# rayglover-ibm/sparse-solvers

Measured on AMD Instinct MI355X. Metric: signals recovered/sec (Homotopy l1, m=8192 n=65536 k=64 fp32), higher is better.
Workload: dtype f32; 1 GPU; configs[1]: one signal per solve, A 8192x65536 fp32 = default_rng(1234).standard_normal/sqrt(m) (SURVEY 8d recipe), k=64 positive coefficients, tol 1e-3, max_iter 256; shipped defaults (reference behaviour: tie_guard 0, zero_on_removal 0); m=8192, n=65536, k=64, sweep_variant=5, engine=1

## Files before the change

### sparse-solvers_amd/csrc/resident.hip

```cpp
#include "ss_hip_internal.h"
#include "ss_hip_device.h"
#include "resident.h"

#include <hip/hip_fp16.h>

#include <algorithm>
#include <cmath>
#include <cstdio>
#include <cstdlib>
#include <cstring>

namespace sship {

template <typename T> struct ResVec;
template <> struct ResVec<double> { typedef double v2 __attribute__((ext_vector_type(2))); };
template <> struct ResVec<float>  { typedef float v2 __attribute__((ext_vector_type(2))); };

template <typename T>
struct ResLds {
    T* I;
    T* dvec;
    T* xvec;
    T* u1sg;
    T* u2w;
    int32_t* posof;
    uint32_t* subc;
    uint32_t* pcol;
    uint32_t* psub;
};

template <typename T>
__host__ __device__ inline size_t res_lds_bytes()
{
    typedef ResCfg<T> C;
    return ((size_t)C::PCAP * (C::PCAP + 1) + 6 * (size_t)C::PCAP) * sizeof(T) + ((size_t)2 * C::S + 2 * (size_t)C::PCAP) * 4;
}

template <typename T> __device__ __forceinline__ T res_sqrt(T v);
template <> __device__ __forceinline__ float res_sqrt<float>(float v) { return sqrtf(v); }
template <> __device__ __forceinline__ double res_sqrt<double>(double v) { return sqrt(v); }
template <typename T> __device__ __forceinline__ T res_fma(T a, T b, T c);
template <> __device__ __forceinline__ float res_fma<float>(float a, float b, float c) { return __builtin_fmaf(a, b, c); }
template <> __device__ __forceinline__ double res_fma<double>(double a, double b, double c) { return __builtin_fma(a, b, c); }
template <typename T> __device__ __forceinline__ T res_abs(T v) { return v < T(0) ? -v : v; }

__device__ __forceinline__ uint32_t uni(uint32_t v) { return (uint32_t)__builtin_amdgcn_readfirstlane((int)v); }
__device__ __forceinline__ int32_t uni(int32_t v) { return __builtin_amdgcn_readfirstlane(v); }
__device__ __forceinline__ float uni(float v) { return __uint_as_float(uni(__float_as_uint(v))); }
__device__ __forceinline__ double uni(double v)
{
    const uint32_t lo = uni((uint32_t)__double2loint(v)), hi = uni((uint32_t)__double2hiint(v));
    return __hiloint2double((int)hi, (int)lo);
}

__device__ __forceinline__ void lds_barrier() { asm volatile("s_waitcnt lgkmcnt(0)\n\ts_barrier" ::: "memory"); }

__device__ __forceinline__ void cmov_inplace(float& dst, float src, unsigned long long msk)
{
    asm volatile("v_cndmask_b32_e64 %0, %0, %1, %2" : "+v"(dst) : "v"(src), "s"(msk));
}
__device__ __forceinline__ void cmov_inplace(double& dst, double src, unsigned long long msk)
{
    uint32_t lo = (uint32_t)__double2loint(dst), hi = (uint32_t)__double2hiint(dst);
    const uint32_t slo = (uint32_t)__double2loint(src), shi = (uint32_t)__double2hiint(src);
    asm volatile("v_cndmask_b32_e64 %0, %0, %2, %4\n\tv_cndmask_b32_e64 %1, %1, %3, %4" : "+v"(lo), "+v"(hi) : "v"(slo), "v"(shi), "s"(msk));
    dst = __hiloint2double((int)hi, (int)lo);
}

template <typename T>
__device__ __forceinline__ T group8_sum(T v)
{
    v += dpp_mov<kDppXor1>(v);
    v += dpp_mov<kDppXor2>(v);
    v += dpp_mov<kDppHalfMirror>(v);
    return v;
}

template <typename T>
__device__ __forceinline__ T wave_max_val(T v)
{
    { const T o = dpp_mov<kDppXor1>(v); v = o > v ? o : v; }
    { const T o = dpp_mov<kDppXor2>(v); v = o > v ? o : v; }
    { const T o = dpp_mov<kDppHalfMirror>(v); v = o > v ? o : v; }
    { const T o = dpp_mov<kDppMirror>(v); v = o > v ? o : v; }
    T b = lane_value(v, 0);
#pragma unroll
    for (int r = 1; r < 4; ++r) { const T o = lane_value(v, 16 * r); b = o > b ? o : b; }
    return b;
}

template <typename T, bool OMP, bool STAMPS = false>
__global__ __launch_bounds__(ResCfg<T>::THREADS)
void k_res_solve(const T* __restrict__ Gs_all, uint32_t gpitch, size_t g_slot_stride, const T* __restrict__ c0_all, uint32_t c0_stride,
                 const uint32_t* __restrict__ sub_all, uint32_t n, T tol, uint32_t max_iter, int strict_sign, int tie_guard, int tie_exit,
                 uint32_t kcap, uint32_t* __restrict__ log_hdr, T* __restrict__ log_H, uint32_t* __restrict__ log_pcol, T* __restrict__ log_X, T* __restrict__ log_D,
                 T* __restrict__ x_all, uint32_t x_stride, uint32_t* __restrict__ gam2_all, uint32_t* __restrict__ touched2_all,
                 DevState* __restrict__ st_all, TraceEntry* trace, uint32_t trace_cap, unsigned long long* dbg = nullptr)
{
    unsigned long long tph[6] = { 0, 0, 0, 0, 0, 0 };
    unsigned long long tlast = 0;
#define RES_STAMP(PH) if constexpr (STAMPS) { const unsigned long long now_ = __builtin_readcyclecounter(); tph[PH] += now_ - tlast; tlast = now_; }
    typedef ResCfg<T> C;
    typedef typename ResVec<T>::v2 V2;
    constexpr uint32_t S = C::S, THREADS = C::THREADS, PCAP = C::PCAP, LOGCAP = C::LOGCAP;
    constexpr int CT = C::CT, PT = C::PCAP / 8;
    constexpr uint32_t NW = (THREADS + 63) / 64;
    constexpr uint32_t IP = PCAP + 1u;
    static_assert(THREADS / 8 * CT == S, "eight lanes per column group");
    static_assert(PCAP % 8 == 0 && (CT == 4 || CT == 8), "positions dealt out over the eight lanes of a group");
    extern __shared__ __attribute__((aligned(16))) unsigned char smem[];
    __shared__ T s_max[16];
    __shared__ T s_minv[16];
    __shared__ uint32_t s_mini[16];
    __shared__ T s_f[4];
    __shared__ uint32_t s_tie;
    ResLds<T> L;
    {
        T* p = reinterpret_cast<T*>(smem);
        L.I = p; p += (size_t)PCAP * IP;
        L.dvec = p; p += PCAP; L.xvec = p; p += PCAP; L.u1sg = p; p += 2 * PCAP; L.u2w = p; p += 2 * PCAP;
        L.posof = reinterpret_cast<int32_t*>(p);
        L.subc = reinterpret_cast<uint32_t*>(L.posof + S);
        L.pcol = L.subc + S;
        L.psub = L.pcol + PCAP;
    }
    const uint32_t slot = blockIdx.x, t = threadIdx.x, lane = t & 63u, wave = t >> 6;
    const uint32_t grp = t >> 3, g = t & 7u;
    const T* Gs = Gs_all + (size_t)slot * g_slot_stride;
    const T* c0 = c0_all + (size_t)slot * c0_stride;
    const uint32_t* sub = sub_all + (size_t)slot * S;
    T* x_out = x_all + (size_t)slot * x_stride;
    uint32_t* gam_out = gam2_all + (size_t)slot * 2 * kcap;
    uint32_t* tch_out = touched2_all + (size_t)slot * 2 * kcap;
    DevState* st = st_all + slot;
    uint32_t* hdr = log_hdr + (size_t)slot * LOGCAP * 8;
    T* LH = log_H != nullptr ? log_H + (size_t)slot * LOGCAP * 2 : nullptr;
    T* LX = log_X + (size_t)slot * LOGCAP * PCAP;
    T* LD = log_D != nullptr ? log_D + (size_t)slot * LOGCAP * PCAP : nullptr;
    if (slot != 0) trace = nullptr;

    const uint32_t jc0 = grp * (uint32_t)CT;
    const bool owner = g < (uint32_t)CT;
    const uint32_t myj = jc0 + (g & (uint32_t)(CT - 1));
    const uint32_t mycol = sub[myj];
    const bool myvalid = owner && mycol < n;
    const T my_c0 = mycol < n ? c0[mycol] : T(0);
    T my_c = my_c0, my_q = T(0);
    T gr[CT][PT];
#pragma unroll
    for (int c = 0; c < CT; ++c)
#pragma unroll
        for (int e = 0; e < PT; ++e) gr[c][e] = T(0);
    for (uint32_t j = t; j < S; j += THREADS) { L.subc[j] = sub[j]; L.posof[j] = -1; }
    for (uint32_t p = t; p < PCAP; p += THREADS) {
        L.dvec[p] = T(0); L.xvec[p] = T(0); L.pcol[p] = 0xffffffffu; L.psub[p] = 0u;
        L.u1sg[2 * p] = T(0); L.u1sg[2 * p + 1] = T(0); L.u2w[2 * p] = T(0); L.u2w[2 * p + 1] = T(0);
    }
    for (uint32_t e = t; e < PCAP * IP; e += THREADS) L.I[e] = T(0);
    if (t == 0) s_tie = 0u;
    T warm = T(0);
    {
        const size_t gbytes = (size_t)S * gpitch * sizeof(T);
        const unsigned char* gb = reinterpret_cast<const unsigned char*>(Gs);
#pragma unroll 4
        for (size_t off = (size_t)t * 128u; off < gbytes; off += (size_t)THREADS * 128u) warm += *reinterpret_cast<const T*>(gb + off);
    }

    auto wave_first = [&](T v, T ext, uint32_t idx) __attribute__((always_inline)) -> uint32_t {
        const unsigned long long bal = __builtin_amdgcn_ballot_w64(v == ext);
        const int src = bal != 0ull ? (int)__builtin_ctzll(bal) : 0;
        return (uint32_t)__builtin_amdgcn_readlane((int)idx, src);
    };
    auto block_min = [&](T& v, uint32_t& i) __attribute__((always_inline)) {
        const T wv = -wave_max_val<T>(-v);
        const uint32_t wi = wave_first(v, wv, i);
        if (lane == 0) { s_minv[wave] = wv; s_mini[wave] = wi; }
        lds_barrier();
        T bv = s_minv[0];
        uint32_t bi = s_mini[0];
#pragma unroll
        for (uint32_t w = 1; w < NW; ++w) {
            const T ov = s_minv[w];
            const uint32_t oi = s_mini[w];
            if (ov < bv) { bv = ov; bi = oi; }
        }
        v = uni(bv); i = uni(bi);
    };
    auto block_argmax = [&](T& v, uint32_t& i) __attribute__((always_inline)) {
        const T wv = wave_max_val<T>(v);
        const uint32_t wi = wave_first(v, wv, i);
        lds_barrier();
        if (lane == 0) { s_minv[wave] = wv; s_mini[wave] = wi; }
        lds_barrier();
        T bv = s_minv[0];
        uint32_t bi = s_mini[0];
#pragma unroll
        for (uint32_t w = 1; w < NW; ++w) {
            const T ov = s_minv[w];
            const uint32_t oi = s_mini[w];
            if (ov > bv) { bv = ov; bi = oi; }
        }
        v = uni(bv); i = uni(bi);
        lds_barrier();
    };
    auto border_inverse = [&](uint32_t P, T dvv) __attribute__((always_inline)) {
        constexpr uint32_t RW = PCAP / 2u + 1u;
        constexpr uint32_t NG = THREADS / RW;
        const uint32_t Pn = P + 1u;
        const uint32_t pa = t % RW, vg = t / RW;
        const uint32_t a0 = pa, a1 = Pn - 1u - pa;
        if (P != 0xffffffffu && vg < NG && 2u * pa < Pn + 1u - 0u && a0 <= a1) {
            const uint32_t n0 = Pn - a0;
            const uint32_t ntot = a0 == a1 ? n0 : n0 + (Pn - a1);
            const T u0 = a0 < P ? L.u2w[2 * a0] : T(0), u1v = a1 < P ? L.u2w[2 * a1] : T(0);
#pragma nounroll
            for (uint32_t k = vg; k < ntot; k += NG) {
                const bool first = k < n0;
                const uint32_t a = first ? a0 : a1;
                const uint32_t b = first ? a0 + k : a1 + (k - n0);
                const T ua = first ? u0 : u1v;
                T val;
                if (b == P) val = a == P ? dvv : -dvv * ua;
                else val = L.I[a * IP + b] + (dvv * ua) * L.u2w[2 * b];
                L.I[a * IP + b] = val;
                L.I[b * IP + a] = val;
            }
        }
    };

    auto enter_row = [&](uint32_t spi, uint32_t Pn, uint32_t pendP, T pend_dv) __attribute__((always_inline)) -> T {
        const T* row = Gs + (size_t)spi * gpitch;
        const T mine_g = row[myj];
        T gv[CT];
        if constexpr (sizeof(T) == 8) {
            const v2d a = *reinterpret_cast<const v2d*>(row + jc0), b = *reinterpret_cast<const v2d*>(row + jc0 + 2);
            gv[0] = a[0]; gv[1] = a[1]; gv[2] = b[0]; gv[3] = b[1];
        } else {
            const v4f a = *reinterpret_cast<const v4f*>(row + jc0), b = *reinterpret_cast<const v4f*>(row + jc0 + 4);
#pragma unroll
            for (int e = 0; e < 4; ++e) { gv[e] = a[e]; gv[4 + e] = b[e]; }
        }
        border_inverse(pendP, pend_dv);
        const uint32_t e_new = uni(Pn >> 3);
        const unsigned long long msk = __builtin_amdgcn_ballot_w64(g == (Pn & 7u));
#pragma unroll
        for (int e = 0; e < PT; ++e) {
            if (e_new == (uint32_t)e) {
#pragma unroll
                for (int c = 0; c < CT; ++c) cmov_inplace(gr[c][e], gv[c], msk);
            }
        }
        return mine_g;
    };
    auto chain = [&](const T* vec, uint32_t P) __attribute__((always_inline)) -> T {
        T acc[CT];
#pragma unroll
        for (int c = 0; c < CT; ++c) acc[c] = T(0);
#pragma unroll
        for (int e = 0; e < PT; ++e) {
            if ((uint32_t)(8 * e) < P) {
                const T dval = vec[8 * e + (int)g];
#pragma unroll
                for (int c = 0; c < CT; ++c) acc[c] = res_fma<T>(dval, gr[c][e], acc[c]);
            }
        }
        T h4[4];
        if constexpr (CT == 8) {
            const bool up = (g & 4u) != 0u;
#pragma unroll
            for (int i = 0; i < 4; ++i) {
                const T keep = up ? acc[4 + i] : acc[i], send = up ? acc[i] : acc[4 + i];
                h4[i] = keep + dpp_mov<kDppHalfMirror>(send);
            }
        } else {
#pragma unroll
            for (int i = 0; i < 4; ++i) h4[i] = acc[i] + dpp_mov<kDppHalfMirror>(acc[i]);
        }
        const bool b1 = (g & 2u) != 0u, b0 = (g & 1u) != 0u;
        const T k0 = (b1 ? h4[2] : h4[0]) + dpp_mov<kDppXor2>(b1 ? h4[0] : h4[2]);
        const T k1 = (b1 ? h4[3] : h4[1]) + dpp_mov<kDppXor2>(b1 ? h4[1] : h4[3]);
        return (b0 ? k1 : k0) + dpp_mov<kDppXor1>(b0 ? k0 : k1);
    };
    auto inverse_pass = [&](uint32_t P) __attribute__((always_inline)) {
        constexpr int CH = sizeof(T) == 8 ? 6 : PT;
        for (uint32_t a = grp; a < P; a += THREADS / 8u) {
            const T* row = L.I + (size_t)a * IP + g;
            const T* us = L.u1sg + 2u * g;
            T s1 = T(0), s2 = T(0);
#pragma nounroll
            for (int e0 = 0; e0 < PT; e0 += CH) {
                if ((uint32_t)(8 * e0) < P) {
                    T iv[CH];
                    V2 pr[CH];
#pragma unroll
                    for (int e = 0; e < CH; ++e) {
                        if (e0 + e < PT) {
                            iv[e] = row[8 * (e0 + e)];
                            pr[e] = *reinterpret_cast<const V2*>(&us[16 * (e0 + e)]);
                        } else { iv[e] = T(0); pr[e] = V2{ T(0), T(0) }; }
                    }
#pragma unroll
                    for (int e = 0; e < CH; ++e) {
                        s1 = res_fma<T>(iv[e], pr[e][0], s1);
                        s2 = res_fma<T>(iv[e], pr[e][1], s2);
                    }
                }
            }
            s1 = group8_sum<T>(s1); s2 = group8_sum<T>(s2);
            if (g == 0) { L.u2w[2 * a] = s1; L.u2w[2 * a + 1] = s2; }
        }
    };
    auto two_dots = [&](uint32_t P, T& d1, T& d2) __attribute__((always_inline)) {
        T a1 = T(0), a2 = T(0);
#pragma nounroll
        for (uint32_t b = lane; b < P; b += 64u) {
            const V2 pr = *reinterpret_cast<const V2*>(&L.u1sg[2 * b]);
            const T u2b = L.u2w[2 * b];
            a1 = res_fma<T>(pr[0], u2b, a1);
            a2 = res_fma<T>(u2b, pr[1], a2);
        }
        d1 = wave_sum<T>(a1); d2 = wave_sum<T>(a2);
    };
    uint32_t P = 0, status = 0, iter = 0, nlog = 0, reason = 0;
    T c_inf = T(0), lambda_prev = T(0), gamma_prev = T(0), lambda0 = T(0);
    int32_t mypos = -1;
    bool tie_any = false;
    lds_barrier();

    uint32_t sp0;
    {
        T bv = myvalid ? res_abs<T>(my_c) : T(-1);
        uint32_t bi = myvalid ? myj : 0xffffffffu;
        block_argmax(bv, bi);
        sp0 = bi;
        lambda0 = bv;
    }
    if (sp0 >= S) { status = kStatusSubsetDecline; reason |= kReasonNoCand; }
    else {
        const T g00 = enter_row(sp0, 0u, 0xffffffffu, T(0));
        if (owner && myj == sp0) {
            const T nrm = res_sqrt<T>(g00);
            const T inv00 = T(1) / (nrm * nrm);
            const T seed = strict_sign ? my_c : res_abs<T>(my_c);
            const T sg0 = sign_tol<T>(seed, tol);
            L.I[0] = inv00;
            if (OMP) L.xvec[0] = inv00 * my_c; else L.dvec[0] = inv00 * sg0;
            L.pcol[0] = mycol; L.psub[0] = sp0; L.posof[sp0] = 0;
            mypos = 0;
            if (!OMP && trace != nullptr) { trace[0].idx = mycol; trace[0].added = 1; trace[0].gamma = 0.0; trace[0].c_inf = (double)res_abs<T>(my_c); }
        }
        P = 1;
        c_inf = lambda0;
        lambda_prev = lambda0;
        if (!((double)tol >= (sizeof(T) == 8 ? kGramGuard64 : kGramGuard) * (double)lambda0)) { status = kStatusSubsetDecline; reason |= kReasonGuard; }
        lds_barrier();
    }

    if constexpr (OMP) {
        if (status == 0u && !(lambda0 > tol)) { status = kStatusSubsetDecline; reason |= kReasonNoCand; }
        if (status == 0u) {
            if (t == 0) {
                uint32_t* h = hdr;
                h[0] = 0u; h[1] = 1u; h[2] = L.subc[sp0]; h[3] = 1u; h[4] = __float_as_uint((float)lambda0); h[5] = 0u; h[6] = 0xffffffffu; h[7] = 0u;
                if (LH != nullptr) { LH[0] = lambda0; LH[1] = T(0); }
                if (trace != nullptr && 1u < trace_cap) { trace[1].idx = L.subc[sp0]; trace[1].added = 1u; trace[1].gamma = 0.0; trace[1].c_inf = (double)lambda0; }
            }
            if (t < PCAP) LX[t] = T(0);
            nlog = 1;
            iter = 1;
        }
        for (uint32_t round = 2; status == 0u; ++round) {
            my_c = my_c0 - chain(L.xvec, P);
            T bv = T(-1);
            uint32_t bi = 0xffffffffu;
            if (myvalid) { bv = res_abs<T>(my_c); bi = myj; }
            block_argmax(bv, bi);
            c_inf = bv;
            const bool stop = !(c_inf > tol) || round > max_iter;
            const bool logfull = nlog >= LOGCAP;
            const uint32_t spi = bi < S ? bi : 0u;
            const bool stall = !stop && (bi >= S || uni(L.posof[spi]) >= 0);
            const bool full = !stop && (P >= PCAP || P + 1u > kcap);
            const bool ok = !stop && !logfull && !stall && !full;
            if (logfull) { status = kStatusSubsetDecline; reason |= kReasonLog; }
            else if (stall) { status = kStatusSubsetDecline; reason |= kReasonNoCand; }
            else if (full) { status = kStatusSubsetDecline; reason |= kReasonPositions; }
            else if (stop) { status = 0xffffffffu; iter = round - 1; }
            const uint32_t idx = uni(L.subc[spi]);
            if (!logfull) {
                if (t == 0) {
                    uint32_t* h = hdr + nlog * 8;
                    h[0] = P; h[1] = stop ? 0u : 1u; h[2] = ok ? idx : 0xffffffffu; h[3] = ok ? 1u : 0u; h[4] = __float_as_uint((float)c_inf); h[5] = 0u;
                    h[6] = 0xffffffffu; h[7] = 0u;
                    if (LH != nullptr) { LH[nlog * 2] = c_inf; LH[nlog * 2 + 1] = T(0); }
                    if (ok && trace != nullptr && round < trace_cap) { trace[round].idx = idx; trace[round].added = 1u; trace[round].gamma = 0.0; trace[round].c_inf = (double)c_inf; }
                }
                if (t < PCAP) LX[(size_t)nlog * PCAP + t] = t < P ? L.xvec[t] : T(0);
                ++nlog;
            }
            const T my_g = enter_row(spi, ok ? P : 0xffffffffu, 0xffffffffu, T(0));
            if (owner && mypos >= 0) { L.u1sg[2 * mypos] = my_g; L.u1sg[2 * mypos + 1] = my_c0; }
            if (ok && owner && myj == spi) { s_f[0] = my_g; s_f[1] = my_c0; L.posof[spi] = (int32_t)P; L.pcol[P] = idx; L.psub[P] = spi; mypos = (int32_t)P; }
            lds_barrier();
            inverse_pass(P);
            lds_barrier();
            T d1, d2;
            two_dots(P, d1, d2);
            const T dvv = T(1) / (s_f[0] - d1);
            const T beta = dvv * (s_f[1] - d2);
            if (ok && t < P) L.xvec[t] = L.u2w[2 * t + 1] - beta * L.u2w[2 * t];
            if (ok && t == P) L.xvec[P] = beta;
            border_inverse(ok ? P : 0xffffffffu, dvv);
            lds_barrier();
            if (ok) { P += 1u; iter = round; }
        }
        if (status == 0xffffffffu) status = 0u;
    } else {
        if (status == 0u) my_q = chain(L.dvec, P);
        uint32_t pendP = 0xffffffffu;
        T pend_dv = T(0);
        for (uint32_t round = 1; status == 0u; ++round) {
            if constexpr (STAMPS) tlast = __builtin_readcyclecounter();
            const bool stop = (round > 1 && !(c_inf > tol)) || round > max_iter;
            const bool logfull = nlog >= LOGCAP;
            const bool in_band = tie_band<T>(c_inf, lambda_prev, gamma_prev, lambda0);
            T m = Lim<T>::max();
            bool tie = false;
            if (myvalid) {
                if (mypos >= 0) {
                    const T tt = -L.xvec[mypos] / L.dvec[mypos];
                    if (tt > T(0) && tt < m) m = tt;
                } else {
                    const T dl = T(1) - my_q, dr = T(1) + my_q;
                    if (dl != T(0)) {
                        T tt = (c_inf - my_c) / dl;
                        if (tie_guard && tt == T(0) && dl > T(0)) tt = Lim<T>::tiny();
                        if (tt == T(0) && in_band) tie = true;
                        if (tt > T(0) && tt < m) m = tt;
                    }
                    if (dr != T(0)) {
                        T tt = (c_inf + my_c) / dr;
                        if (tie_guard && tt == T(0) && dr > T(0)) tt = Lim<T>::tiny();
                        if (tt == T(0) && in_band) tie = true;
                        if (tt > T(0) && tt < m) m = tt;
                    }
                }
            }
            if (tie) s_tie = 1u;
            T gmm = m;
            uint32_t bi = myvalid ? myj : 0xffffffffu;
            block_min(gmm, bi);
            RES_STAMP(0)
            if (!stop) tie_any = uni(s_tie) != 0u || tie_any;
            const uint32_t spi = bi < S ? bi : 0u;
            const bool tied = !stop && tie_any && tie_exit != 0;
            const bool nocand = !stop && !tied && (bi >= S || !(gmm < Lim<T>::max()));
            const bool leaves = !stop && !tied && !nocand && uni(L.posof[spi]) >= 0;
            const bool full = !stop && !tied && !nocand && !leaves && (P >= PCAP || P + 1u > kcap);
            const bool ok = !stop && !logfull && !tied && !nocand && !leaves && !full;
            if (logfull) { status = kStatusSubsetDecline; reason |= kReasonLog; }
            else if (stop) { status = 0xffffffffu; iter = round - 1; }
            else if (tied) { status = kStatusTieRerun; reason |= kReasonTie; iter = round - 1; }
            else if (nocand) { status = kStatusSubsetDecline; reason |= kReasonNoCand; }
            else if (leaves) { status = kStatusSubsetDecline; reason |= kReasonRemoval; }
            else if (full) { status = kStatusSubsetDecline; reason |= kReasonPositions; }
            const uint32_t idx = uni(L.subc[spi]);
            if (!logfull) {
                if (t == 0) {
                    uint32_t* h = hdr + nlog * 8;
                    h[0] = P; h[1] = stop ? 0u : 1u; h[2] = ok ? idx : 0xffffffffu; h[3] = ok ? 1u : 0u; h[4] = __float_as_uint((float)c_inf);
                    h[5] = ok ? __float_as_uint((float)gmm) : 0u; h[6] = 0xffffffffu; h[7] = in_band ? 1u : 0u;
                    if (LH != nullptr) { LH[nlog * 2] = c_inf; LH[nlog * 2 + 1] = ok ? gmm : T(0); }
                    if (ok && trace != nullptr && round < trace_cap) { trace[round].idx = idx; trace[round].added = 1u; trace[round].gamma = (double)gmm; trace[round].c_inf = (double)c_inf; }
                }
                if (t < PCAP) {
                    LX[(size_t)nlog * PCAP + t] = t < P ? L.xvec[t] : T(0);
                    if (LD != nullptr) LD[(size_t)nlog * PCAP + t] = t < P ? L.dvec[t] : T(0);
                }
                if (stop || tied || ok) ++nlog;
            }
            const T my_g = enter_row(spi, ok ? P : 0xffffffffu, pendP, pend_dv);
            pendP = 0xffffffffu;
            if (ok && t < P) L.xvec[t] = L.xvec[t] + gmm * L.dvec[t];
            if (ok) my_c = res_fma<T>(-gmm, my_q, my_c);
            {
                const T mx = wave_max_val<T>(myvalid ? res_abs<T>(my_c) : T(-1));
                if (lane == 0) s_max[wave] = mx;
            }
            if (owner && mypos >= 0) { L.u1sg[2 * mypos] = my_g; L.u1sg[2 * mypos + 1] = sign_tol<T>(my_c, tol); }
            if (ok && owner && myj == spi) {
                s_f[0] = my_g; s_f[1] = sign_tol<T>(my_c, tol);
                L.posof[spi] = (int32_t)P; L.pcol[P] = idx; L.psub[P] = spi; mypos = (int32_t)P;
            }
            lds_barrier();
            RES_STAMP(1)
            T c_next = s_max[0];
#pragma unroll
            for (uint32_t w = 1; w < NW; ++w) { const T o = s_max[w]; c_next = o > c_next ? o : c_next; }
            c_next = uni(c_next);
            if (t == 0) s_tie = 0u;
            inverse_pass(P);
            lds_barrier();
            RES_STAMP(2)
            T d1, d2;
            two_dots(P, d1, d2);
            const T dvv = T(1) / (s_f[0] - d1);
            const T beta = dvv * (s_f[1] - d2);
            if (ok && t < P) L.dvec[t] = L.u2w[2 * t + 1] - beta * L.u2w[2 * t];
            if (ok && t == P) L.dvec[P] = beta;
            pendP = ok ? P : 0xffffffffu;
            pend_dv = dvv;
            lds_barrier();
            RES_STAMP(3)
            if (ok) {
                P += 1u;
                lambda_prev = c_inf;
                gamma_prev = gmm;
                c_inf = c_next;
                iter = round;
            }
            my_q = chain(L.dvec, P);
            RES_STAMP(4)
            if constexpr (STAMPS) tph[5] += 1;
        }
        if (status == 0xffffffffu) status = 0u;
    }
    if constexpr (STAMPS) {
        if (dbg != nullptr && slot == 0u && t == 0u)
            for (int q = 0; q < 6; ++q) dbg[q] = tph[q];
    }
#undef RES_STAMP
    lds_barrier();
    if (t < PCAP) log_pcol[(size_t)slot * PCAP + t] = t < P ? L.pcol[t] : 0xffffffffu;
    if (status == 0u || status == kStatusTieRerun) {
        if (t < P) {
            const uint32_t col = L.pcol[t];
            uint32_t rk = 0;
#pragma nounroll
            for (uint32_t b = 0; b < P; ++b) rk += L.pcol[b] < col ? 1u : 0u;
            gam_out[rk] = col;
            tch_out[rk] = col;
            x_out[col] = L.xvec[t];
        }
    }
    if (t == 0) {
        st->done = 1;
        st->status = status;
        st->iter = iter;
        st->K = P;
        st->ntouched = P;
        st->cur = 0;
        st->c_inf = (double)c_inf;
        st->gamma = (double)gamma_prev;
        st->tie_stall = tie_any ? 1u : 0u;
        st->lambda0 = (float)lambda0;
        st->solo_nlog = nlog;
        st->need_sweep = 0;
        st->done_round = iter + 1u;
        st->sub_reason = reason;
    }
    if (warm == T(1.2345e-30)) st->pad4_[0] = 1u;
}

constexpr uint32_t kG64T = 64, kG64Step = 32, kG64Pitch = kG64Step + 1;
typedef double res_v4d __attribute__((ext_vector_type(4)));

__global__ __launch_bounds__(256)
void k_sgram64_part(const double* __restrict__ At, uint32_t ldm, uint32_t n, const uint32_t* __restrict__ sub, uint32_t rows_per,
                    double* __restrict__ part)
{
    constexpr uint32_t S = ResCfg<double>::S;
    __shared__ double sI[kG64T][kG64Pitch];
    __shared__ double sJ[kG64T][kG64Pitch];
    sub += (size_t)blockIdx.z * S;
    part += (size_t)blockIdx.z * gridDim.y * S * S;
    const uint32_t b = blockIdx.x;
    uint32_t tt = (uint32_t)((__fsqrt_rn(8.f * (float)b + 1.f) - 1.f) * 0.5f);
    while (tt * (tt + 1u) / 2u > b) --tt;
    while ((tt + 1u) * (tt + 2u) / 2u <= b) ++tt;
    const uint32_t bj = tt, bi = b - tt * (tt + 1u) / 2u;
    const uint32_t chunk = blockIdx.y;
    const uint32_t tid = threadIdx.x, lane = tid & 63u, w = tid >> 6;
    const uint32_t wi = w >> 1, wj = w & 1u;
    const uint32_t sc = tid >> 2, sq = tid & 3u;
    const uint32_t ci = sub[bi * kG64T + sc], cj = sub[bj * kG64T + sc];
    const bool oki = ci < n, okj = cj < n;
    const double* gi = At + (size_t)(oki ? ci : 0u) * ldm + (size_t)chunk * rows_per + 8u * sq;
    const double* gj = At + (size_t)(okj ? cj : 0u) * ldm + (size_t)chunk * rows_per + 8u * sq;
    const v2d zero2 = { 0.0, 0.0 };
    v2d vi[4], vj[4];
#define SG64_LOAD(R0)                                                                         \
    _Pragma("unroll") for (int p = 0; p < 4; ++p) {                                           \
        vi[p] = oki ? *reinterpret_cast<const v2d*>(gi + (R0) + 2 * p) : zero2;               \
        vj[p] = okj ? *reinterpret_cast<const v2d*>(gj + (R0) + 2 * p) : zero2;               \
    }
    SG64_LOAD(0u)
    res_v4d acc[2][2];
#pragma unroll
    for (int i = 0; i < 2; ++i)
#pragma unroll
        for (int j = 0; j < 2; ++j) acc[i][j] = res_v4d{ 0.0, 0.0, 0.0, 0.0 };
    const uint32_t l15 = lane & 15u, kq = lane >> 4;
    for (uint32_t r0 = 0; r0 < rows_per; r0 += kG64Step) {
        __syncthreads();
#pragma unroll
        for (int p = 0; p < 4; ++p) {
            sI[sc][8u * sq + 2u * (uint32_t)p] = vi[p][0]; sI[sc][8u * sq + 2u * (uint32_t)p + 1u] = vi[p][1];
            sJ[sc][8u * sq + 2u * (uint32_t)p] = vj[p][0]; sJ[sc][8u * sq + 2u * (uint32_t)p + 1u] = vj[p][1];
        }
        __syncthreads();
        if (r0 + kG64Step < rows_per) SG64_LOAD(r0 + kG64Step)
#pragma unroll
        for (uint32_t k4 = 0; k4 < kG64Step; k4 += 4) {
            const double a0 = sI[32u * wi + l15][k4 + kq], a1 = sI[32u * wi + 16u + l15][k4 + kq];
            const double b0 = sJ[32u * wj + l15][k4 + kq], b1 = sJ[32u * wj + 16u + l15][k4 + kq];
            acc[0][0] = __builtin_amdgcn_mfma_f64_16x16x4f64(a0, b0, acc[0][0], 0, 0, 0);
            acc[0][1] = __builtin_amdgcn_mfma_f64_16x16x4f64(a0, b1, acc[0][1], 0, 0, 0);
            acc[1][0] = __builtin_amdgcn_mfma_f64_16x16x4f64(a1, b0, acc[1][0], 0, 0, 0);
            acc[1][1] = __builtin_amdgcn_mfma_f64_16x16x4f64(a1, b1, acc[1][1], 0, 0, 0);
        }
    }
#undef SG64_LOAD
    double* Pp = part + (size_t)chunk * S * S;
#pragma unroll
    for (int i = 0; i < 2; ++i)
#pragma unroll
        for (int j = 0; j < 2; ++j)
#pragma unroll
            for (int e = 0; e < 4; ++e) {
                const uint32_t row = bi * kG64T + 32u * wi + 16u * (uint32_t)i + 4u * (uint32_t)e + kq;
                const uint32_t col = bj * kG64T + 32u * wj + 16u * (uint32_t)j + l15;
                Pp[(size_t)row * S + col] = acc[i][j][e];
                if (bi != bj) Pp[(size_t)col * S + row] = acc[i][j][e];
            }
}

__global__ __launch_bounds__(256)
void k_sgram64_sum(const double* __restrict__ part, uint32_t nsplit, double* __restrict__ gs, const double* __restrict__ At, uint32_t ldm,
                   const double* __restrict__ y, const uint32_t* __restrict__ sub, uint32_t n, double* __restrict__ c0, uint32_t c0_stride)
{
    constexpr uint32_t S = ResCfg<double>::S;
    constexpr uint32_t NB = S * S / 256u;
    {
        const size_t slot = blockIdx.y;
        part += slot * nsplit * S * S; gs += slot * S * S; y += slot * ldm; sub += slot * S; c0 += slot * c0_stride;
    }
    if (blockIdx.x >= NB) {
        __shared__ double sv[16];
        const uint32_t col = sub[blockIdx.x - NB];
        const double* a = At + (size_t)(col < n ? col : 0u) * ldm;
        double acc = 0.0;
        for (uint32_t r0 = 2u * threadIdx.x; r0 < ldm; r0 += 8u * 512u) {
            v2d av[8], yv[8];
// ... 78 lines not shown
    }
    const uint32_t Pfin = hdr[(size_t)(nlog - 1u) * 8u];
    if (tid < kR64Rhs) {
        float sc = 1.f;
        if (tid < nst) {
            const double lam = LH[(size_t)(tid + 1u) * 2u];
            const bool final_state = !(hdr[(size_t)(tid + 1u) * 8u + 1u] & 1u);
            sc = res_state_scale((float)(final_state ? fmax(lam, tol) : lam));
        }
        sS[tid] = sc;
    }
    const uint32_t rg = tid & 15u, sgp = tid >> 4;
    double acc[3][4][4];
    {
        const v2d y0 = *reinterpret_cast<const v2d*>(y + r0 + 4u * rg), y1 = *reinterpret_cast<const v2d*>(y + r0 + 4u * rg + 2u);
#pragma unroll
        for (int rd = 0; rd < 3; ++rd)
#pragma unroll
            for (int si = 0; si < 4; ++si) { acc[rd][si][0] = y0[0]; acc[rd][si][1] = y0[1]; acc[rd][si][2] = y1[0]; acc[rd][si][3] = y1[1]; }
    }
    for (uint32_t u0 = 0; u0 < Pfin; u0 += 16u) {
        __syncthreads();
        {
            const uint32_t p = tid >> 4, q4 = tid & 15u;
            const uint32_t u = u0 + p;
            const uint32_t col = u < Pfin ? pcol[u] : 0xffffffffu;
            v2d a0 = { 0.0, 0.0 }, a1 = { 0.0, 0.0 };
            if (col < n) {
                a0 = *reinterpret_cast<const v2d*>(At + (size_t)col * ldm + r0 + 4u * q4);
                a1 = *reinterpret_cast<const v2d*>(At + (size_t)col * ldm + r0 + 4u * q4 + 2u);
            }
            *reinterpret_cast<v2d*>(&sAc[p][4u * q4]) = a0;
            *reinterpret_cast<v2d*>(&sAc[p][4u * q4 + 2u]) = a1;
            for (uint32_t e = tid; e < 16u * XP; e += 256u) {
                const uint32_t k = e / 16u, pp = e - k * 16u;
                sXt[pp][k] = (u0 + pp < Pfin && k < nst) ? LX[(size_t)(k + 1u) * PCAP + u0 + pp] : 0.0;
            }
        }
        __syncthreads();
#pragma unroll
        for (int rd = 0; rd < 3; ++rd) {
            const uint32_t s0 = 64u * (uint32_t)rd + 4u * sgp;
            if (s0 < nst) {
#pragma unroll 4
                for (uint32_t p = 0; p < 16u; ++p) {
                    const v2d a0 = *reinterpret_cast<const v2d*>(&sAc[p][4u * rg]), a1 = *reinterpret_cast<const v2d*>(&sAc[p][4u * rg + 2u]);
                    const v2d x0 = *reinterpret_cast<const v2d*>(&sXt[p][s0]), x1 = *reinterpret_cast<const v2d*>(&sXt[p][s0 + 2u]);
                    const double av[4] = { a0[0], a0[1], a1[0], a1[1] }, xv[4] = { x0[0], x0[1], x1[0], x1[1] };
#pragma unroll
                    for (int si = 0; si < 4; ++si)
#pragma unroll
                        for (int ri = 0; ri < 4; ++ri) acc[rd][si][ri] = __builtin_fma(-xv[si], av[ri], acc[rd][si][ri]);
                }
            }
        }
    }
    bool ovf = false;
#pragma unroll
    for (int rd = 0; rd < 3; ++rd) {
#pragma unroll
        for (int si = 0; si < 4; ++si) {
            const uint32_t kk = 64u * (uint32_t)rd + 4u * sgp + (uint32_t)si;
            const float sc = sS[kk < kR64Rhs ? kk : 0u];
            float ss = 0.f;
            __half hv[4];
#pragma unroll
            for (int ri = 0; ri < 4; ++ri) {
                const float r = (float)acc[rd][si][ri];
                ss = __builtin_fmaf(r, r, ss);
                const float v = r * sc;
                if (kk < nst && !(fabsf(v) < 60000.f)) ovf = true;
                hv[ri] = __float2half_rn(v);
            }
            ss += __shfl_xor(ss, 1); ss += __shfl_xor(ss, 2); ss += __shfl_xor(ss, 4); ss += __shfl_xor(ss, 8);
            if (kk < nst) {
                *reinterpret_cast<uint2*>(r16 + (size_t)kk * ldm + r0 + 4u * rg) = *reinterpret_cast<const uint2*>(hv);
                if (rg == 0u) rn2p[(size_t)blockIdx.x * kR64Rhs + kk] = ss * 1.0001f;
            }
        }
    }
    if (ovf && !scan) { __hip_atomic_store(&st->need_sweep, 1u, __ATOMIC_RELAXED, __HIP_MEMORY_SCOPE_AGENT); atomicOr(&st->sub_reason, kReasonOverflow); }
    if (blockIdx.x == 0u) {
        if (tid == 0u && blockIdx.y == 0u) *headroom = __float_as_uint(ratio0);
        if (tid < nst) {
            const uint32_t* hh = hdr + (size_t)(tid + 1u) * 8u;
            const uint32_t* hp = hdr + (size_t)tid * 8u;
            const double lam_d = LH[(size_t)(tid + 1u) * 2u];
            const double lam_pd = LH[(size_t)tid * 2u], gam_pd = LH[(size_t)tid * 2u + 1u];
            const float lam = (float)lam_d;
            const bool final_state = !(hh[1] & 1u);
            const float slack = 1e-12f * (float)LH[0];
            float bound;
            if (omp) {
                bound = (final_state && !(lam_d > tol) ? (float)tol * 0.9375f : lam * 0.875f) - slack;
            } else {
                const double lam_exp = lam_pd - gam_pd;
                const bool ls_jump = final_state && !(lam_d > tol) && !(lam_exp > 1e-13 * LH[0]);
                if (ls_jump) bound = (float)tol * 0.9375f - slack;
                else bound = fminf(lam, (float)lam_exp) * 0.875f - slack;
                const bool irregular = hp[3] == 0u || lam_d > lam_pd * (1.0 + 1e-12);
                if (irregular && !scan) {
                    bound = -1.f;
                    atomicOr(&st->sub_reason, kReasonIrregular);
                    __hip_atomic_store(&st->need_sweep, 1u, __ATOMIC_RELAXED, __HIP_MEMORY_SCOPE_AGENT);
                }
                if (scan && (irregular || final_state)) bound = 3.0e38f;
            }
            const float inv_sk = 1.f / sS[tid];
            tab[tid * 4u + 0] = meta[1] * inv_sk;
            tab[tid * 4u + 1] = bound;
            tab[tid * 4u + 2] = inv_sk;
            tab[tid * 4u + 3] = lam;
        }
    }
}

template <typename T>
bool res_solve_usable()
{
    static const bool ok = [] {
        const hipError_t e = hipFuncSetAttribute(reinterpret_cast<const void*>(&k_res_solve<T, false>), hipFuncAttributeMaxDynamicSharedMemorySize,
                                                 (int)res_lds_bytes<T>());
        const hipError_t e2 = hipFuncSetAttribute(reinterpret_cast<const void*>(&k_res_solve<T, true>), hipFuncAttributeMaxDynamicSharedMemorySize,
                                                  (int)res_lds_bytes<T>());
        if (e != hipSuccess || e2 != hipSuccess) (void)hipGetLastError();
        return e == hipSuccess && e2 == hipSuccess;
    }();
    return ok;
}
template bool res_solve_usable<float>();
template bool res_solve_usable<double>();

template <typename T>
hipError_t launch_res_solve(ss_hip_ctx* ctx, uint32_t nslots, const T* Gs, uint32_t gpitch, size_t g_slot_stride, const T* c0, uint32_t c0_stride,
                            const uint32_t* sub, T tol, uint32_t max_iter, uint32_t kcap, const ResLog<T>& log, T* x, uint32_t x_stride,
                            uint32_t* gam2, uint32_t* touched2, DevState* st, TraceEntry* trace, uint32_t trace_cap, bool omp)
{
    if (!res_solve_usable<T>()) return hipErrorInvalidConfiguration;
    static unsigned long long* dbg = nullptr;
    static const bool stamps = std::getenv("SS_HIP_RES_STAMPS") != nullptr;
    if (stamps && !omp) {
        static const bool ok = [] {
            const bool a = hipFuncSetAttribute(reinterpret_cast<const void*>(&k_res_solve<T, false, true>), hipFuncAttributeMaxDynamicSharedMemorySize,
                                               (int)res_lds_bytes<T>()) == hipSuccess;
            return a && hipMalloc(&dbg, 8 * sizeof(unsigned long long)) == hipSuccess;
        }();
        if (ok) {
            hipLaunchKernelGGL((k_res_solve<T, false, true>), dim3(nslots), dim3(ResCfg<T>::THREADS), res_lds_bytes<T>(), ctx->stream, Gs, gpitch, g_slot_stride, c0, c0_stride,
                               sub, (uint32_t)ctx->n, tol, max_iter, ctx->strict_sign, ctx->tie_guard, (ctx->tie_rerun && !ctx->tie_guard) ? 1 : 0, kcap,
                               log.hdr, log.H, log.pcol, log.X, log.D, x, x_stride, gam2, touched2, st, trace, trace_cap, dbg);
            unsigned long long tp[6];
            if (hipMemcpyAsync(tp, dbg, sizeof(tp), hipMemcpyDeviceToHost, ctx->stream) == hipSuccess && hipStreamSynchronize(ctx->stream) == hipSuccess) {
                const double r = tp[5] ? (double)tp[5] : 1.0;
                std::fprintf(stderr, "[k_res_solve<%s>, cycles per round over %llu rounds] scan+argmin %.0f  row+x+c %.0f  inverse pass %.0f  dots+dir+border %.0f  chain %.0f\n",
                             sizeof(T) == 8 ? "double" : "float", tp[5], tp[0] / r, tp[1] / r, tp[2] / r, tp[3] / r, tp[4] / r);
            }
            return hipGetLastError();
        }
    }
    if (omp)
        hipLaunchKernelGGL((k_res_solve<T, true>), dim3(nslots), dim3(ResCfg<T>::THREADS), res_lds_bytes<T>(), ctx->stream, Gs, gpitch, g_slot_stride, c0, c0_stride,
                           sub, (uint32_t)ctx->n, tol, max_iter, ctx->strict_sign, ctx->tie_guard, (ctx->tie_rerun && !ctx->tie_guard) ? 1 : 0, kcap,
                           log.hdr, log.H, log.pcol, log.X, log.D, x, x_stride, gam2, touched2, st, trace, trace_cap);
    else
        hipLaunchKernelGGL((k_res_solve<T, false>), dim3(nslots), dim3(ResCfg<T>::THREADS), res_lds_bytes<T>(), ctx->stream, Gs, gpitch, g_slot_stride, c0, c0_stride,
                           sub, (uint32_t)ctx->n, tol, max_iter, ctx->strict_sign, ctx->tie_guard, (ctx->tie_rerun && !ctx->tie_guard) ? 1 : 0, kcap,
                           log.hdr, log.H, log.pcol, log.X, log.D, x, x_stride, gam2, touched2, st, trace, trace_cap);
    return hipGetLastError();
}
template hipError_t launch_res_solve<float>(ss_hip_ctx*, uint32_t, const float*, uint32_t, size_t, const float*, uint32_t, const uint32_t*, float, uint32_t,
                                            uint32_t, const ResLog<float>&, float*, uint32_t, uint32_t*, uint32_t*, DevState*, TraceEntry*, uint32_t, bool);
template hipError_t launch_res_solve<double>(ss_hip_ctx*, uint32_t, const double*, uint32_t, size_t, const double*, uint32_t, const uint32_t*, double, uint32_t,
                                             uint32_t, const ResLog<double>&, double*, uint32_t, uint32_t*, uint32_t*, DevState*, TraceEntry*, uint32_t, bool);

hipError_t launch_sgram64(ss_hip_ctx* ctx, const uint32_t* sub, const double* y, double* part, double* gs, double* c0, uint32_t nslots, uint32_t c0_stride)
{
    constexpr uint32_t S = ResCfg<double>::S, NT = S / kG64T;
    const uint32_t ldm = ctx->ldm;
    uint32_t nsplit = ldm / 512u;
    if (nsplit == 0u || ldm % (nsplit * kG64Step) != 0u) nsplit = ldm / 256u;
    if (nsplit > kSg64MaxSplit) nsplit = kSg64MaxSplit;
    while (nsplit > 1u && ldm % (nsplit * kG64Step) != 0u) --nsplit;
    const double* At = static_cast<const double*>(ctx->At);
    hipLaunchKernelGGL(k_sgram64_part, dim3(NT * (NT + 1) / 2, nsplit, nslots), dim3(256), 0, ctx->stream, At, ldm, (uint32_t)ctx->n, sub, ldm / nsplit, part);
    hipLaunchKernelGGL(k_sgram64_sum, dim3(S * S / 256u + S, nslots), dim3(256), 0, ctx->stream, (const double*)part, nsplit, gs, At, ldm, y, sub, (uint32_t)ctx->n, c0,
                       c0_stride);
    return hipGetLastError();
}

hipError_t launch_res_residuals64(ss_hip_ctx* ctx, const double* y, const ResLog<double>& log, double tol, const float* meta, void* r16, float* rn2p,
                                  float* tab, uint32_t* headroom, DevState* st, bool first16, bool omp, uint32_t nslots, const float* slotmeta, uint32_t* fl, bool scan)
{
    hipLaunchKernelGGL(k_res_residuals64, dim3(ctx->ldm / 64u, nslots), dim3(256), 0, ctx->stream, static_cast<const double*>(ctx->At), ctx->ldm, (uint32_t)ctx->n, y,
                       (const uint32_t*)log.hdr, (const double*)log.H, (const uint32_t*)log.pcol, (const double*)log.X, tol, meta,
                       static_cast<__half*>(r16), rn2p, tab, headroom, st, first16 ? 1 : 0, omp ? 1 : 0, slotmeta, fl, scan ? 1 : 0);
    return hipGetLastError();
}

}
```

Measured before the change: 1621 signals/s.

## Fold pick metadata into block reductions and overlap row fetch with border update

Block min/argmax reductions now publish a 16-byte record per wave holding the value, subset index, position and tie flag. This removes the separate shared-memory reads of posof, subc and the s_tie flag that followed each reduction. The next Gram row is loaded right after the reduction, before the branch-free verdict logic and the border inverse update, so its global latency overlaps with that work. The border inverse loop is batched (2 or 3 elements) to issue more LDS reads before the writes, and the log stores reuse x/d values already loaded into registers. In exchange the control flow is more intricate, and the asm barriers pin registers, which may raise register pressure.

```diff
diff --git a/sparse-solvers_amd/csrc/resident.hip b/sparse-solvers_amd/csrc/resident.hip
--- a/sparse-solvers_amd/csrc/resident.hip
+++ b/sparse-solvers_amd/csrc/resident.hip
@@ -88,6 +88,10 @@
     for (int r = 1; r < 4; ++r) { const T o = lane_value(v, 16 * r); b = o > b ? o : b; }
     return b;
 }
+
+constexpr uint32_t kPickNone = 0xffffu;
+template <typename T> struct alignas(16) ResPick { T v; uint32_t who; uint32_t col; };
+static_assert(sizeof(ResPick<float>) == 16 && sizeof(ResPick<double>) == 16, "one 16-byte read per wave");
 
 template <typename T, bool OMP, bool STAMPS = false>
 __global__ __launch_bounds__(ResCfg<T>::THREADS)
@@ -110,10 +114,8 @@
     static_assert(PCAP % 8 == 0 && (CT == 4 || CT == 8), "positions dealt out over the eight lanes of a group");
     extern __shared__ __attribute__((aligned(16))) unsigned char smem[];
     __shared__ T s_max[16];
-    __shared__ T s_minv[16];
-    __shared__ uint32_t s_mini[16];
+    __shared__ ResPick<T> s_pick[NW];
     __shared__ T s_f[4];
-    __shared__ uint32_t s_tie;
     ResLds<T> L;
     {
         T* p = reinterpret_cast<T*>(smem);
@@ -146,6 +148,7 @@
     const bool myvalid = owner && mycol < n;
     const T my_c0 = mycol < n ? c0[mycol] : T(0);
     T my_c = my_c0, my_q = T(0);
+    int32_t mypos = -1;
     T gr[CT][PT];
 #pragma unroll
     for (int c = 0; c < CT; ++c)
@@ -157,7 +160,6 @@
         L.u1sg[2 * p] = T(0); L.u1sg[2 * p + 1] = T(0); L.u2w[2 * p] = T(0); L.u2w[2 * p + 1] = T(0);
     }
     for (uint32_t e = t; e < PCAP * IP; e += THREADS) L.I[e] = T(0);
-    if (t == 0) s_tie = 0u;
     T warm = T(0);
     {
         const size_t gbytes = (size_t)S * gpitch * sizeof(T);
@@ -166,41 +168,48 @@
         for (size_t off = (size_t)t * 128u; off < gbytes; off += (size_t)THREADS * 128u) warm += *reinterpret_cast<const T*>(gb + off);
     }
 
-    auto wave_first = [&](T v, T ext, uint32_t idx) __attribute__((always_inline)) -> uint32_t {
+    auto publish_pick = [&](T v, T ext, bool tiew) __attribute__((always_inline)) {
         const unsigned long long bal = __builtin_amdgcn_ballot_w64(v == ext);
-        const int src = bal != 0ull ? (int)__builtin_ctzll(bal) : 0;
-        return (uint32_t)__builtin_amdgcn_readlane((int)idx, src);
+        const uint32_t src = bal != 0ull ? (uint32_t)__builtin_ctzll(bal) : 0u;
+        if (lane == src) {
+            ResPick<T> sl;
+            sl.v = ext;
+            sl.who = (myvalid ? myj : kPickNone) | ((uint32_t)(mypos + 1) << 16) | (tiew ? 0x80000000u : 0u);
+            sl.col = mycol;
+            s_pick[wave] = sl;
+        }
     };
-    auto block_min = [&](T& v, uint32_t& i) __attribute__((always_inline)) {
-        const T wv = -wave_max_val<T>(-v);
-        const uint32_t wi = wave_first(v, wv, i);
-        if (lane == 0) { s_minv[wave] = wv; s_mini[wave] = wi; }
+    auto gather_pick = [&](bool want_min, T& v, uint32_t& i, uint32_t& col, int32_t& pos, bool& tie) __attribute__((always_inline)) {
+        ResPick<T> sl[NW];
+#pragma unroll
+        for (uint32_t w = 0; w < NW; ++w) sl[w] = s_pick[w];
+        T bv = sl[0].v;
+        uint32_t bw = sl[0].who, bc = sl[0].col, ties = sl[0].who;
+#pragma unroll
+        for (uint32_t w = 1; w < NW; ++w) {
+            const bool take = want_min ? sl[w].v < bv : sl[w].v > bv;
+            bv = take ? sl[w].v : bv; bw = take ? sl[w].who : bw; bc = take ? sl[w].col : bc;
+            ties |= sl[w].who;
+        }
+        v = uni(bv);
+        const uint32_t who = uni((bw & 0x7fffffffu) | (ties & 0x80000000u));
+        col = uni(bc);
+        i = (who & 0xffffu) == kPickNone ? 0xffffffffu : (who & 0xffffu);
+        pos = (int32_t)((who >> 16) & 0x7fffu) - 1;
+        tie = (who >> 31) != 0u;
+    };
+    auto block_min = [&](T m, bool tie, T& v, uint32_t& i, uint32_t& col, int32_t& pos, bool& anytie) __attribute__((always_inline)) {
+        publish_pick(m, -wave_max_val<T>(-m), __builtin_amdgcn_ballot_w64(tie) != 0ull);
         lds_barrier();
-        T bv = s_minv[0];
-        uint32_t bi = s_mini[0];
-#pragma unroll
-        for (uint32_t w = 1; w < NW; ++w) {
-            const T ov = s_minv[w];
-            const uint32_t oi = s_mini[w];
-            if (ov < bv) { bv = ov; bi = oi; }
-        }
-        v = uni(bv); i = uni(bi);
+        gather_pick(true, v, i, col, pos, anytie);
     };
-    auto block_argmax = [&](T& v, uint32_t& i) __attribute__((always_inline)) {
-        const T wv = wave_max_val<T>(v);
-        const uint32_t wi = wave_first(v, wv, i);
+    auto block_argmax = [&](T m, T& v, uint32_t& i, uint32_t& col, int32_t& pos) __attribute__((always_inline)) {
+        const T wv = wave_max_val<T>(m);
         lds_barrier();
-        if (lane == 0) { s_minv[wave] = wv; s_mini[wave] = wi; }
+        publish_pick(m, wv, false);
         lds_barrier();
-        T bv = s_minv[0];
-        uint32_t bi = s_mini[0];
-#pragma unroll
-        for (uint32_t w = 1; w < NW; ++w) {
-            const T ov = s_minv[w];
-            const uint32_t oi = s_mini[w];
-            if (ov > bv) { bv = ov; bi = oi; }
-        }
-        v = uni(bv); i = uni(bi);
+        bool none;
+        gather_pick(false, v, i, col, pos, none);
         lds_barrier();
     };
     auto border_inverse = [&](uint32_t P, T dvv) __attribute__((always_inline)) {
@@ -213,44 +222,75 @@
             const uint32_t n0 = Pn - a0;
             const uint32_t ntot = a0 == a1 ? n0 : n0 + (Pn - a1);
             const T u0 = a0 < P ? L.u2w[2 * a0] : T(0), u1v = a1 < P ? L.u2w[2 * a1] : T(0);
+            constexpr uint32_t BU = sizeof(T) == 8 ? 2u : 3u;
+            auto where = [&](uint32_t k, uint32_t& a, uint32_t& b, T& ua) __attribute__((always_inline)) {
+                const bool first = k < n0;
+                a = first ? a0 : a1;
+                b = first ? a0 + k : a1 + (k - n0);
+                ua = first ? u0 : u1v;
+            };
+            auto value = [&](uint32_t a, uint32_t b, T ua, T iv, T ub) __attribute__((always_inline)) -> T {
+                const T edge = a == P ? dvv : -dvv * ua;
+                const T inner = iv + (dvv * ua) * ub;
+                return b == P ? edge : inner;
+            };
+            uint32_t k = vg;
 #pragma nounroll
-            for (uint32_t k = vg; k < ntot; k += NG) {
-                const bool first = k < n0;
-                const uint32_t a = first ? a0 : a1;
-                const uint32_t b = first ? a0 + k : a1 + (k - n0);
-                const T ua = first ? u0 : u1v;
-                T val;
-                if (b == P) val = a == P ? dvv : -dvv * ua;
-                else val = L.I[a * IP + b] + (dvv * ua) * L.u2w[2 * b];
-                L.I[a * IP + b] = val;
-                L.I[b * IP + a] = val;
+            for (; k + (BU - 1u) * NG < ntot; k += BU * NG) {
+                uint32_t ea[BU], eb[BU];
+                T ua[BU], iv[BU], ub[BU];
+#pragma unroll
+                for (uint32_t u = 0; u < BU; ++u) {
+                    where(k + u * NG, ea[u], eb[u], ua[u]);
+                    iv[u] = L.I[ea[u] * IP + eb[u]];
+                    ub[u] = L.u2w[2 * eb[u]];
+                }
+#pragma unroll
+                for (uint32_t u = 0; u < BU; ++u) {
+                    const T val = value(ea[u], eb[u], ua[u], iv[u], ub[u]);
+                    L.I[ea[u] * IP + eb[u]] = val;
+                    L.I[eb[u] * IP + ea[u]] = val;
+                }
+            }
+#pragma nounroll
+            for (; k < ntot; k += NG) {
+                uint32_t ea, eb;
+                T ua;
+                where(k, ea, eb, ua);
+                const T val = value(ea, eb, ua, L.I[ea * IP + eb], L.u2w[2 * eb]);
+                L.I[ea * IP + eb] = val;
+                L.I[eb * IP + ea] = val;
             }
         }
     };
 
-    auto enter_row = [&](uint32_t spi, uint32_t Pn, uint32_t pendP, T pend_dv) __attribute__((always_inline)) -> T {
+    struct RowVals { T mine; T gv[CT]; };
+    auto row_fetch = [&](uint32_t spi, RowVals& rv) __attribute__((always_inline)) {
         const T* row = Gs + (size_t)spi * gpitch;
-        const T mine_g = row[myj];
-        T gv[CT];
+        rv.mine = row[myj];
         if constexpr (sizeof(T) == 8) {
             const v2d a = *reinterpret_cast<const v2d*>(row + jc0), b = *reinterpret_cast<const v2d*>(row + jc0 + 2);
-            gv[0] = a[0]; gv[1] = a[1]; gv[2] = b[0]; gv[3] = b[1];
+            rv.gv[0] = a[0]; rv.gv[1] = a[1]; rv.gv[2] = b[0]; rv.gv[3] = b[1];
         } else {
             const v4f a = *reinterpret_cast<const v4f*>(row + jc0), b = *reinterpret_cast<const v4f*>(row + jc0 + 4);
 #pragma unroll
-            for (int e = 0; e < 4; ++e) { gv[e] = a[e]; gv[4 + e] = b[e]; }
-        }
-        border_inverse(pendP, pend_dv);
+            for (int e = 0; e < 4; ++e) { rv.gv[e] = a[e]; rv.gv[4 + e] = b[e]; }
+        }
+        asm volatile("" ::: "memory");
+    };
+    auto row_place = [&](uint32_t Pn, const RowVals& rv) __attribute__((always_inline)) {
         const uint32_t e_new = uni(Pn >> 3);
         const unsigned long long msk = __builtin_amdgcn_ballot_w64(g == (Pn & 7u));
 #pragma unroll
+        for (int c = 0; c < CT; ++c) asm volatile("" :: "v"(rv.gv[c]));
+        asm volatile("" :: "v"(rv.mine));
+#pragma unroll
         for (int e = 0; e < PT; ++e) {
             if (e_new == (uint32_t)e) {
 #pragma unroll
-                for (int c = 0; c < CT; ++c) cmov_inplace(gr[c][e], gv[c], msk);
-            }
-        }
-        return mine_g;
+                for (int c = 0; c < CT; ++c) cmov_inplace(gr[c][e], rv.gv[c], msk);
+            }
+        }
     };
     auto chain = [&](const T* vec, uint32_t P) __attribute__((always_inline)) -> T {
         T acc[CT];
@@ -321,23 +361,24 @@
         }
         d1 = wave_sum<T>(a1); d2 = wave_sum<T>(a2);
     };
+    asm volatile("" : "+s"(trace_cap));
     uint32_t P = 0, status = 0, iter = 0, nlog = 0, reason = 0;
     T c_inf = T(0), lambda_prev = T(0), gamma_prev = T(0), lambda0 = T(0);
-    int32_t mypos = -1;
     bool tie_any = false;
     lds_barrier();
 
     uint32_t sp0;
     {
-        T bv = myvalid ? res_abs<T>(my_c) : T(-1);
-        uint32_t bi = myvalid ? myj : 0xffffffffu;
-        block_argmax(bv, bi);
-        sp0 = bi;
-        lambda0 = bv;
+        uint32_t col0;
+        int32_t pos0;
+        block_argmax(myvalid ? res_abs<T>(my_c) : T(-1), lambda0, sp0, col0, pos0);
     }
     if (sp0 >= S) { status = kStatusSubsetDecline; reason |= kReasonNoCand; }
     else {
-        const T g00 = enter_row(sp0, 0u, 0xffffffffu, T(0));
+        RowVals rv0;
+        row_fetch(sp0, rv0);
+        row_place(0u, rv0);
+        const T g00 = rv0.mine;
         if (owner && myj == sp0) {
             const T nrm = res_sqrt<T>(g00);
             const T inv00 = T(1) / (nrm * nrm);
@@ -371,22 +412,30 @@
         }
         for (uint32_t round = 2; status == 0u; ++round) {
             my_c = my_c0 - chain(L.xvec, P);
-            T bv = T(-1);
-            uint32_t bi = 0xffffffffu;
-            if (myvalid) { bv = res_abs<T>(my_c); bi = myj; }
-            block_argmax(bv, bi);
-            c_inf = bv;
+            uint32_t bi, idx;
+            int32_t wpos;
+            block_argmax(myvalid ? res_abs<T>(my_c) : T(-1), c_inf, bi, idx, wpos);
+            const uint32_t spi = bi < S ? bi : 0u;
+            RowVals rv;
+            row_fetch(spi, rv);
             const bool stop = !(c_inf > tol) || round > max_iter;
             const bool logfull = nlog >= LOGCAP;
-            const uint32_t spi = bi < S ? bi : 0u;
-            const bool stall = !stop && (bi >= S || uni(L.posof[spi]) >= 0);
-            const bool full = !stop && (P >= PCAP || P + 1u > kcap);
-            const bool ok = !stop && !logfull && !stall && !full;
-            if (logfull) { status = kStatusSubsetDecline; reason |= kReasonLog; }
-            else if (stall) { status = kStatusSubsetDecline; reason |= kReasonNoCand; }
-            else if (full) { status = kStatusSubsetDecline; reason |= kReasonPositions; }
-            else if (stop) { status = 0xffffffffu; iter = round - 1; }
-            const uint32_t idx = uni(L.subc[spi]);
+            const bool stall_c = bi >= S || wpos >= 0;
+            const bool full_c = P >= PCAP || P + 1u > kcap;
+            uint32_t verdict = full_c ? kReasonPositions : 0u;
+            verdict = stall_c ? (uint32_t)kReasonNoCand : verdict;
+            verdict = stop ? 0u : verdict;
+            verdict = logfull ? (uint32_t)kReasonLog : verdict;
+            const bool ok = !stop && verdict == 0u;
+            const bool ends = stop && !logfull;
+            status = verdict != 0u ? (uint32_t)kStatusSubsetDecline : ends ? 0xffffffffu : status;
+            reason |= verdict;
+            iter = ends ? round - 1 : iter;
+            row_place(ok ? P : 0xffffffffu, rv);
+            const T my_g = rv.mine;
+            if (owner && mypos >= 0) { L.u1sg[2 * mypos] = my_g; L.u1sg[2 * mypos + 1] = my_c0; }
+            if (ok && owner && myj == spi) { s_f[0] = my_g; s_f[1] = my_c0; L.posof[spi] = (int32_t)P; L.pcol[P] = idx; L.psub[P] = spi; mypos = (int32_t)P; }
+            lds_barrier();
             if (!logfull) {
                 if (t == 0) {
                     uint32_t* h = hdr + nlog * 8;
@@ -398,10 +447,6 @@
                 if (t < PCAP) LX[(size_t)nlog * PCAP + t] = t < P ? L.xvec[t] : T(0);
                 ++nlog;
             }
-            const T my_g = enter_row(spi, ok ? P : 0xffffffffu, 0xffffffffu, T(0));
-            if (owner && mypos >= 0) { L.u1sg[2 * mypos] = my_g; L.u1sg[2 * mypos + 1] = my_c0; }
-            if (ok && owner && myj == spi) { s_f[0] = my_g; s_f[1] = my_c0; L.posof[spi] = (int32_t)P; L.pcol[P] = idx; L.psub[P] = spi; mypos = (int32_t)P; }
-            lds_barrier();
             inverse_pass(P);
             lds_barrier();
             T d1, d2;
@@ -419,6 +464,8 @@
         if (status == 0u) my_q = chain(L.dvec, P);
         uint32_t pendP = 0xffffffffu;
         T pend_dv = T(0);
+        constexpr uint32_t TL0 = THREADS - ((PCAP + 63u) / 64u) * 64u;
+        const uint32_t tl = t - TL0;
         for (uint32_t round = 1; status == 0u; ++round) {
             if constexpr (STAMPS) tlast = __builtin_readcyclecounter();
             const bool stop = (round > 1 && !(c_inf > tol)) || round > max_iter;
@@ -446,59 +493,68 @@
                     }
                 }
             }
-            if (tie) s_tie = 1u;
-            T gmm = m;
-            uint32_t bi = myvalid ? myj : 0xffffffffu;
-            block_min(gmm, bi);
+            T gmm;
+            uint32_t bi, idx;
+            int32_t wpos;
+            bool anytie;
+            block_min(m, tie, gmm, bi, idx, wpos, anytie);
             RES_STAMP(0)
-            if (!stop) tie_any = uni(s_tie) != 0u || tie_any;
             const uint32_t spi = bi < S ? bi : 0u;
-            const bool tied = !stop && tie_any && tie_exit != 0;
-            const bool nocand = !stop && !tied && (bi >= S || !(gmm < Lim<T>::max()));
-            const bool leaves = !stop && !tied && !nocand && uni(L.posof[spi]) >= 0;
-            const bool full = !stop && !tied && !nocand && !leaves && (P >= PCAP || P + 1u > kcap);
-            const bool ok = !stop && !logfull && !tied && !nocand && !leaves && !full;
-            if (logfull) { status = kStatusSubsetDecline; reason |= kReasonLog; }
-            else if (stop) { status = 0xffffffffu; iter = round - 1; }
-            else if (tied) { status = kStatusTieRerun; reason |= kReasonTie; iter = round - 1; }
-            else if (nocand) { status = kStatusSubsetDecline; reason |= kReasonNoCand; }
-            else if (leaves) { status = kStatusSubsetDecline; reason |= kReasonRemoval; }
-            else if (full) { status = kStatusSubsetDecline; reason |= kReasonPositions; }
-            const uint32_t idx = uni(L.subc[spi]);
+            RowVals rv;
+            row_fetch(spi, rv);
+            tie_any = tie_any || (!stop && anytie);
+            const bool tied_c = tie_any && tie_exit != 0;
+            const bool nocand_c = bi >= S || !(gmm < Lim<T>::max());
+            const bool full_c = P >= PCAP || P + 1u > kcap;
+            uint32_t verdict = full_c ? kReasonPositions : 0u;
+            verdict = wpos >= 0 ? (uint32_t)kReasonRemoval : verdict;
+            verdict = nocand_c ? (uint32_t)kReasonNoCand : verdict;
+            verdict = tied_c ? (uint32_t)kReasonTie : verdict;
+            verdict = stop ? 0u : verdict;
+            verdict = logfull ? (uint32_t)kReasonLog : verdict;
+            const bool ok = !stop && verdict == 0u;
+            const bool ends = stop && !logfull;
+            const bool tied = verdict == kReasonTie;
+            status = ends ? 0xffffffffu : tied ? (uint32_t)kStatusTieRerun : verdict != 0u ? (uint32_t)kStatusSubsetDecline : status;
+            reason |= verdict;
+            iter = ends || tied ? round - 1 : iter;
+            T xv = T(0), dv = T(0);
+            if (tl < P) { xv = L.xvec[tl]; dv = L.dvec[tl]; }
+            border_inverse(pendP, pend_dv);
+            pendP = 0xffffffffu;
+            if (ok && tl < P) L.xvec[tl] = xv + gmm * dv;
+            if (ok) my_c = res_fma<T>(-gmm, my_q, my_c);
+            {
+                const T mx = wave_max_val<T>(myvalid ? res_abs<T>(my_c) : T(-1));
+                if (lane == 0) s_max[wave] = mx;
+            }
+            row_place(ok ? P : 0xffffffffu, rv);
+            const T my_g = rv.mine;
+            if (owner && mypos >= 0) { L.u1sg[2 * mypos] = my_g; L.u1sg[2 * mypos + 1] = sign_tol<T>(my_c, tol); }
+            if (ok && owner && myj == spi) {
+                s_f[0] = my_g; s_f[1] = sign_tol<T>(my_c, tol);
+                L.posof[spi] = (int32_t)P; L.pcol[P] = idx; L.psub[P] = spi; mypos = (int32_t)P;
+            }
+            lds_barrier();
+            RES_STAMP(1)
             if (!logfull) {
-                if (t == 0) {
+                if (tl == 0u) {
                     uint32_t* h = hdr + nlog * 8;
                     h[0] = P; h[1] = stop ? 0u : 1u; h[2] = ok ? idx : 0xffffffffu; h[3] = ok ? 1u : 0u; h[4] = __float_as_uint((float)c_inf);
                     h[5] = ok ? __float_as_uint((float)gmm) : 0u; h[6] = 0xffffffffu; h[7] = in_band ? 1u : 0u;
                     if (LH != nullptr) { LH[nlog * 2] = c_inf; LH[nlog * 2 + 1] = ok ? gmm : T(0); }
                     if (ok && trace != nullptr && round < trace_cap) { trace[round].idx = idx; trace[round].added = 1u; trace[round].gamma = (double)gmm; trace[round].c_inf = (double)c_inf; }
                 }
-                if (t < PCAP) {
-                    LX[(size_t)nlog * PCAP + t] = t < P ? L.xvec[t] : T(0);
-                    if (LD != nullptr) LD[(size_t)nlog * PCAP + t] = t < P ? L.dvec[t] : T(0);
+                if (tl < PCAP) {
+                    LX[(size_t)nlog * PCAP + tl] = xv;
+                    if (LD != nullptr) LD[(size_t)nlog * PCAP + tl] = dv;
                 }
                 if (stop || tied || ok) ++nlog;
             }
-            const T my_g = enter_row(spi, ok ? P : 0xffffffffu, pendP, pend_dv);
-            pendP = 0xffffffffu;
-            if (ok && t < P) L.xvec[t] = L.xvec[t] + gmm * L.dvec[t];
-            if (ok) my_c = res_fma<T>(-gmm, my_q, my_c);
-            {
-                const T mx = wave_max_val<T>(myvalid ? res_abs<T>(my_c) : T(-1));
-                if (lane == 0) s_max[wave] = mx;
-            }
-            if (owner && mypos >= 0) { L.u1sg[2 * mypos] = my_g; L.u1sg[2 * mypos + 1] = sign_tol<T>(my_c, tol); }
-            if (ok && owner && myj == spi) {
-                s_f[0] = my_g; s_f[1] = sign_tol<T>(my_c, tol);
-                L.posof[spi] = (int32_t)P; L.pcol[P] = idx; L.psub[P] = spi; mypos = (int32_t)P;
-            }
-            lds_barrier();
-            RES_STAMP(1)
             T c_next = s_max[0];
 #pragma unroll
             for (uint32_t w = 1; w < NW; ++w) { const T o = s_max[w]; c_next = o > c_next ? o : c_next; }
             c_next = uni(c_next);
-            if (t == 0) s_tie = 0u;
             inverse_pass(P);
             lds_barrier();
             RES_STAMP(2)
@@ -883,7 +939,7 @@
             unsigned long long tp[6];
             if (hipMemcpyAsync(tp, dbg, sizeof(tp), hipMemcpyDeviceToHost, ctx->stream) == hipSuccess && hipStreamSynchronize(ctx->stream) == hipSuccess) {
                 const double r = tp[5] ? (double)tp[5] : 1.0;
-                std::fprintf(stderr, "[k_res_solve<%s>, cycles per round over %llu rounds] scan+argmin %.0f  row+x+c %.0f  inverse pass %.0f  dots+dir+border %.0f  chain %.0f\n",
+                std::fprintf(stderr, "[k_res_solve<%s>, cycles per round over %llu rounds] scan+argmin %.0f  row+border+x+c %.0f  log+inverse pass %.0f  dots+dir %.0f  chain %.0f\n",
                              sizeof(T) == 8 ? "double" : "float", tp[5], tp[0] / r, tp[1] / r, tp[2] / r, tp[3] / r, tp[4] / r);
             }
             return hipGetLastError();
```

Measured after the change: 1671 signals/s (median of 6 runs). 3.1% higher.
